# ruanjue/smartdenovo

Hardware: AMD Instinct MI355X
Metric: Gbp of candidate pairs aligned/sec (wtzmo all-vs-all) (higher is better)
Workload: dtype int32/int16

## Files before the change

smartdenovo_amd/csrc/wtz_tasks.h:

```cpp
#ifndef WTZ_TASKS_H
#define WTZ_TASKS_H

#include "wtz_sw.h"
#include "wtz_sw_wave.h"
#include "wtz_sw_grp.h"
#include "wtz_sw_lane.h"
#include "wtz_dotmatrix.h"

typedef struct {
	wtz_reads_t R; wtz_zindex_t Z; const wtz_params_t *P; wtz_pool_t *pool;
	wtz_zindex_t ZQ;
	uint32_t dm_first_big;
} wtz_env_t;

#define WTZ_WAVE_LDS_BYTES 8192
#ifndef WTZ_GAP_LDS_BYTES
#define WTZ_GAP_LDS_BYTES 12288
#endif
#ifndef WTZ_PAIR_LDS_BYTES
#define WTZ_PAIR_LDS_BYTES 8192
#endif
#ifndef WTZ_PAIR_DM_LDS_BYTES
#define WTZ_PAIR_DM_LDS_BYTES 24576
#endif
#if defined(__HIP_DEVICE_COMPILE__)
WTZ_D int32_t *wtz_wave_scratch(){ extern __shared__ int32_t wtz_dyn_lds[]; return wtz_dyn_lds; }
#else
WTZ_COOP_HOST int32_t *wtz_wave_scratch(){ return NULL; }
#endif

#if defined(WTZ_DEBUG_CRUMBS) && defined(__HIPCC__)
__device__ unsigned int *wtz_crumbs = NULL;
#endif
#if defined(WTZ_DEBUG_CRUMBS) && defined(__HIP_DEVICE_COMPILE__)
#define WTZ_CRUMB(t, code) do { if(wtz_crumbs && WTZ_LANE == 0) __hip_atomic_store(&wtz_crumbs[t], (unsigned int)(code), __ATOMIC_RELAXED, __HIP_MEMORY_SCOPE_SYSTEM); } while(0)
#else
#define WTZ_CRUMB(t, code) do { } while(0)
#endif
#define WTZ_PAIR_NEEDS_ZBIG (-3)
template<int ENGINE = -1, bool ZBIG = true>
WTZ_HD void wtz_task_pair(uint32_t t, const wtz_env_t &V, const uint32_t *qid, const uint32_t *cid, wtz_pairres_t *res){
	const wtz_params_t *P = V.P;
	const bool dm = ENGINE < 0 ? (P->dot_matrix != 0) : (ENGINE == 1);
	const uint32_t q = qid[t], c = cid[t];
	wtz_pairres_t r; memset(&r, 0, sizeof r);
	wtz_zhit_t *hits = NULL; uint32_t n = 0;
#if defined(__HIP_DEVICE_COMPILE__)
#define WTZ_TICK() ((uint64_t)clock64())
#else
#define WTZ_TICK() ((uint64_t)0)
#endif
	const uint64_t tk0 = WTZ_TICK();
	WTZ_CRUMB(t, 1);
	const bool aux = P->aux_strand != 0;
#if defined(__HIP_DEVICE_COMPILE__)
	const bool ok0 = wtz_zmatch_coop(V.ZQ, V.Z, q, c, V.R.rdlen[c], P->max_kmer_var, V.pool, &hits, &n, aux, (uint32_t*)wtz_wave_scratch(), dm ? (uint32_t)WTZ_PAIR_DM_LDS_BYTES : (uint32_t)WTZ_PAIR_LDS_BYTES);
#else
	const bool ok0 = wtz_zmatch_coop(V.ZQ, V.Z, q, c, V.R.rdlen[c], P->max_kmer_var, V.pool, &hits, &n, aux);
#endif
	const bool ok = wtz_coop_bcast32(ok0 ? 1u : 0u) != 0;
	n = wtz_coop_bcast32(n);
	hits = (wtz_zhit_t*)(uintptr_t)wtz_coop_bcast64((uint64_t)(uintptr_t)hits);
	const uint64_t tk1 = WTZ_TICK();
	WTZ_CRUMB(t, 2 | (n << 8));
	wtz_zhit_t *sorted = NULL;
#if defined(__HIP_DEVICE_COMPILE__)
	__threadfence_block();
	if(ok && (aux ? n > 0 : n * P->zsize >= P->ztot)){
		int pbad = 0;
		if(dm) sorted = wtz_sort_hits_wave<1>(hits, n, V.pool, (uint64_t*)wtz_wave_scratch(), WTZ_PAIR_DM_LDS_BYTES / 8, &pbad);
		else              sorted = wtz_sort_hits_wave<0>(hits, n, V.pool, (uint64_t*)wtz_wave_scratch(), WTZ_PAIR_LDS_BYTES / 8, &pbad);
		if(wtz_coop_bcast32((uint32_t)pbad)) r.bad = 1;
		sorted = (wtz_zhit_t*)(uintptr_t)wtz_coop_bcast64((uint64_t)(uintptr_t)sorted);
	}
#endif
	const uint32_t lane = WTZ_LANE;
	WTZ_CRUMB(t, 3 | (n << 8));
	if(!ok || r.bad){ r.bad = 1; if(lane == 0) res[t] = r; WTZ_CRUMB(t, 0xFF); return; }
	r.n_hits = n;
	if(aux ? n == 0 : n * P->zsize < P->ztot){ r.gate = 0; if(lane == 0) res[t] = r; WTZ_CRUMB(t, 0xFF); return; }
	r.gate = 1;
	if(dm){
		wtz_vec<wtz_zhit_t> cache; cache.a = sorted ? sorted : hits; cache.n = n; cache.cap = n + 2; cache.pool = V.pool; cache.bad = 0;
		const uint64_t tk2 = WTZ_TICK();
		uint64_t tkd = 0;
#if defined(__HIP_DEVICE_COMPILE__)
		uint8_t *dlds = (uint8_t*)wtz_wave_scratch();
#else
		static thread_local uint64_t emul_dm_lds[WTZ_PAIR_DM_LDS_BYTES / 8];
		uint8_t *dlds = (uint8_t*)emul_dm_lds;
#endif
		wtz_dm_result_t d = wtz_dot_matrix_align(cache, V.pool, (int32_t)V.R.rdlen[q], (int32_t)V.R.rdlen[c], P, &r.bad, sorted != NULL, &tkd, dlds, WTZ_PAIR_DM_LDS_BYTES, true, V.dm_first_big != 0);
		if(lane != 0) return;
		if(d.dir == -2){ r.anchors[0] = cache.a; r.nanchors[0] = cache.n; }
		r.dm_score = d.score; r.dm_qb = d.qb; r.dm_qe = d.qe; r.dm_tb = d.tb; r.dm_te = d.te; r.dm_dir = d.dir;
		{ const uint64_t tk3 = WTZ_TICK(); r.tick[0] = (uint32_t)((tk1 - tk0) >> 10); r.tick[1] = (uint32_t)((tk2 - tk1) >> 10); r.tick[2] = (uint32_t)((tkd - tk2) >> 10); r.tick[3] = (uint32_t)((tk3 - tk0) >> 10); }
		res[t] = r; return;
	}
	if(sorted) hits = sorted;
	else { WTZ_CRUMB(t, 4 | (n << 8)); if(lane == 0) wtz_sort_exact(hits, (size_t)n, wtz_gt_off12()); WTZ_WAVE_SYNC(); }
	WTZ_CRUMB(t, 5 | (n << 8));
	const uint64_t tk2 = WTZ_TICK();
	wtz_winscratch_t sc;
	{
		uint64_t pa = 0;
		if(lane == 0) pa = (uint64_t)(uintptr_t)wtz_pool_alloc(V.pool, (size_t)(n + 2) * (4 * 7 + 8 + sizeof(wtz_zhit_t)) + 16);
		pa = wtz_coop_bcast64(pa);
		sc.ts = (uint32_t*)(uintptr_t)pa;
	}
	if(sc.ts == NULL){ r.bad = 1; if(lane == 0) res[t] = r; WTZ_CRUMB(t, 0xFF); return; }
	sc.as = (int32_t*)(sc.ts + (n + 2)); sc.wb = sc.ts + 2 * (n + 2); sc.we = sc.ts + 3 * (n + 2); sc.wo = sc.ts + 4 * (n + 2); sc.wf = sc.ts + 5 * (n + 2); sc.wd = sc.ts + 6 * (n + 2);
	sc.tk = (uint64_t*)(sc.ts + 7 * (n + 2) + ((7 * (n + 2)) & 1)); sc.ztmp = (wtz_zhit_t*)(sc.tk + (n + 2));
#if defined(__HIP_DEVICE_COMPILE__)
	sc.lds = (uint64_t*)wtz_wave_scratch();
#else
	static thread_local uint64_t emul_lds[WTZ_PAIR_LDS_BYTES / 8];
	sc.lds = emul_lds;
#endif
	sc.lds_u64 = WTZ_PAIR_LDS_BYTES / 8;
	sc.big = NULL; sc.big_u64 = 0; sc.need_big = 0;
#ifndef WTZ_MERGE_SCALAR
	wtz_merge_prepare(hits, n, sc, P->kwin);
#endif
	for(uint32_t dir = 0; dir < 2; dir++){
		wtz_vec<wtz_win_t> wins; wtz_vec<wtz_zhit_t> anchors;
		wins.a = NULL; wins.n = wins.cap = 0; wins.pool = V.pool; wins.bad = 0;
		anchors.a = NULL; anchors.n = anchors.cap = 0; anchors.pool = V.pool; anchors.bad = 0;
		if(lane == 0){ wins.init(V.pool, 16); anchors.init(V.pool, n + 16); }
		WTZ_CRUMB(t, (6 + dir) | (n << 8));
		const unsigned long long ptm = WTZ_PROF_T(); (void)ptm;
#ifdef WTZ_MERGE_SCALAR
		const uint32_t nw = wtz_merge_windows_coop<ZBIG>(hits, n, dir, wins, anchors, sc, P->zsize, P->kwin, P->kstep, P->zovl);
#else
		const uint32_t nw = wtz_merge_windows_wave<ZBIG>(hits, n, dir, wins, anchors, sc, P->zsize, P->kwin, P->kstep, P->zovl);
#endif
		WTZ_PROF_ADD(63, ptm);
		if(!ZBIG && sc.need_big){
			if(lane == 0){ wtz_pairres_t r2; memset(&r2, 0, sizeof r2); r2.n_hits = r.n_hits; r2.gate = 1; r2.dm_dir = WTZ_PAIR_NEEDS_ZBIG; res[t] = r2; }
			WTZ_CRUMB(t, 0xFF);
			return;
		}
		WTZ_CRUMB(t, (8 + dir) | (n << 8));
		if(wtz_coop_bcast32((uint32_t)(wins.bad | anchors.bad))){ r.bad = 1; continue; }
		if(nw == 0) continue;
		const unsigned long long ptc = WTZ_PROF_T(); (void)ptc;
		WTZ_WAVE_SYNC();
		const uint32_t wn = wtz_coop_bcast32(wins.n);
		wtz_win_t *wa = (wtz_win_t*)(uintptr_t)wtz_coop_bcast64((uint64_t)(uintptr_t)wins.a);
		int32_t *mem = NULL;
		if(wn > 64u || WTZ_NLANES == 1u){
			uint64_t pa = 0;
			if(lane == 0) pa = (uint64_t)(uintptr_t)wtz_pool_alloc(V.pool, (size_t)wn * 8 + 8);
			mem = (int32_t*)(uintptr_t)wtz_coop_bcast64(pa);
			if(mem == NULL){ r.bad = 1; continue; }
		}
		r.ovl[dir] = WTZ_OVL29(wtz_chain_windows_wave(wa, wn, P->W, mem));
		if(r.ovl[dir] < P->ztot) continue;
		const uint32_t k = wtz_keep_chain_members(wa, wn);
		r.nwin[dir] = k; r.win[dir] = wa; r.anchors[dir] = anchors.a; r.nanchors[dir] = anchors.n;
		WTZ_PROF_ADD(62, ptc);
	}
	if(lane != 0) return;
	{ const uint64_t tk3 = WTZ_TICK(); r.tick[0] = (uint32_t)((tk1 - tk0) >> 10); r.tick[1] = (uint32_t)((tk2 - tk1) >> 10); r.tick[2] = (uint32_t)((tk3 - tk2) >> 10); r.tick[3] = (uint32_t)((tk3 - tk0) >> 10); }
	res[t] = r;
	WTZ_CRUMB(t, 0xFF);
}

WTZ_HD void wtz_task_pair_dm_big(uint32_t t, const wtz_env_t &V, const uint32_t *list, const uint32_t *qid, const uint32_t *cid, wtz_pairres_t *res, uint32_t lds_bytes, bool last, bool big){
	const wtz_params_t *P = V.P;
	const uint32_t pi = list[t], q = qid[pi], c = cid[pi];
	wtz_pairres_t r = res[pi];
	wtz_vec<wtz_zhit_t> cache; cache.a = r.anchors[0]; cache.n = r.nanchors[0]; cache.cap = cache.n + 2; cache.pool = V.pool; cache.bad = 0;
	uint64_t tkd = 0;
#if defined(__HIP_DEVICE_COMPILE__)
	uint8_t *dlds = (uint8_t*)wtz_wave_scratch();
	wtz_dm_result_t d = wtz_dot_matrix_align(cache, V.pool, (int32_t)V.R.rdlen[q], (int32_t)V.R.rdlen[c], P, &r.bad, true, &tkd, dlds, lds_bytes, !last, big);
#else
	(void)lds_bytes; (void)last; (void)big;
	wtz_dm_result_t d = wtz_dot_matrix_align(cache, V.pool, (int32_t)V.R.rdlen[q], (int32_t)V.R.rdlen[c], P, &r.bad, true, &tkd, (uint8_t*)NULL, 0, false, false);
#endif
	if(WTZ_LANE != 0) return;
	r.dm_score = d.score; r.dm_qb = d.qb; r.dm_qe = d.qe; r.dm_tb = d.tb; r.dm_te = d.te; r.dm_dir = d.dir;
	res[pi] = r;
}

typedef struct {
	uint32_t item;
	uint32_t widx;
} wtz_wintask_t;

typedef struct { wtz_aln_t x; uint32_t *cigar; uint32_t cigar_len; uint32_t pass; unsigned long long cells; } wtz_reg_t;

typedef struct {
	uint32_t q, c, dir;
	const wtz_win_t *win; const wtz_zhit_t *anchors; uint32_t nwin;
	wtz_reg_t *regs;
} wtz_alnitem_t;

typedef struct {
	wtz_aln_t x; uint32_t n_regs; uint32_t cigar_len; uint32_t *cigar; int32_t bad;
	unsigned long long cells_shift, cells_fixed, cells_global;
	uint32_t text_len;
} wtz_alnres_dev_t;

WTZ_HD uint32_t wtz_cigar_text_len(const uint32_t *c, uint32_t n){
	uint32_t k = 0;
	for(uint32_t i = 0; i < n; i++){ uint32_t len = c[i] >> 4; if(len == 0) continue; uint32_t d = 1; while(len >= 10){ len /= 10; d++; } k += d + 1; }
	return k;
}
WTZ_HD void wtz_cigar_text_write(const uint32_t *c, uint32_t n, char *s){
	uint32_t k = 0;
// ... 959 lines not shown
```

smartdenovo_amd/csrc/wtz_window.h:

```cpp
#ifndef WTZ_WINDOW_H
#define WTZ_WINDOW_H

#include "wtz_seed.h"

#define WTZ_KWIN_MAX_OFFSET_DEV 50

WTZ_HD bool wtz_zmatch(const wtz_zindex_t &ZQ, const wtz_zindex_t &ZC, uint32_t q, uint32_t c, uint32_t clen, uint32_t max_var, wtz_vec<wtz_zhit_t> &out, bool same_strand = false){
	const uint64_t qo = ZQ.zoff[q], co = ZC.zoff[c];
	const uint32_t cn = (uint32_t)(ZC.zoff[c + 1] - co), qd = ZQ.dn[q];
	const uint32_t *dmer = ZQ.dmer + qo;
	for(uint32_t k = 0; k < cn; k++){
		if(!ZC.ok[co + k]) continue;
		uint32_t m = ZC.mer[co + k];
		uint32_t lo = 0, hi = qd;
		while(lo < hi){ uint32_t mid = (lo + hi) >> 1; if(dmer[mid] < m) lo = mid + 1; else hi = mid; }
		if(lo >= qd || dmer[lo] != m) continue;
		uint32_t cpos = ZC.pos[co + k], clen2 = ZC.len[co + k];
		uint32_t first = ZQ.dfirst[qo + lo], cnt = ZQ.dcnt[qo + lo];
		for(uint32_t e = 0; e < cnt; e++){
			uint32_t qi = ZQ.sidx[qo + first + e];
			uint32_t qpos = ZQ.pos[qo + qi], qlen = ZQ.len[qo + qi];
			uint32_t dv = qlen > clen2 ? qlen - clen2 : clen2 - qlen;
			if(dv > max_var) continue;
			uint32_t d1 = qpos & 1u, d2 = cpos & 1u;
// ... 124 lines not shown
			}
			total += tot;
		}
	}
	if(lane == 0){ wtz_zhit_t z0; z0.o1 = z0.o2 = z0.ll = z0.gid = 0; hits[total] = z0; hits[total + 1] = z0; }
	*out = hits; *n_out = total;
	return true;
}

struct wtz_gt_off12 { WTZ_HDM bool operator()(const wtz_zhit_t &a, const wtz_zhit_t &b) const {
	uint64_t ka = ((uint64_t)ZH_OFF1(a) << 32) | ZH_OFF2(a), kb = ((uint64_t)ZH_OFF1(b) << 32) | ZH_OFF2(b); return ka > kb; } };
struct wtz_gt_off1 { WTZ_HDM bool operator()(const wtz_zhit_t &a, const wtz_zhit_t &b) const { return ZH_OFF1(a) > ZH_OFF1(b); } };
struct wtz_gt_idx_off2 { const wtz_zhit_t *rs; WTZ_HDM bool operator()(uint32_t a, uint32_t b) const { return ZH_OFF2(rs[a]) > ZH_OFF2(rs[b]); } };

#if defined(__HIP_DEVICE_COMPILE__)
template<int SH> struct wtz_gt_keybits { WTZ_HDM bool operator()(uint64_t a, uint64_t b) const { return (a >> SH) > (b >> SH); } };
template<int BYDIAG, bool W_LDS>
WTZ_D wtz_zhit_t *wtz_sort_hits_body(const wtz_zhit_t *hits, uint32_t n, wtz_pool_t *pool, uint64_t *lds, uint32_t lds_u64, uint64_t *w_pool, uint32_t np, int *pool_bad){
	const uint32_t lane = WTZ_LANE;
	const int SH = BYDIAG ? 15 : 16;
	uint64_t *w = W_LDS ? lds : w_pool;
	for(uint32_t i = lane; i < np; i += 64){
		uint64_t v = ~0ull;
		if(i < n){
			if(BYDIAG) v = ((uint64_t)((int64_t)ZH_OFF1(hits[i]) - (int64_t)ZH_OFF2(hits[i]) + (1 << 24)) << 39) | ((uint64_t)ZH_OFF1(hits[i]) << 15) | i;
			else       v = ((uint64_t)ZH_OFF1(hits[i]) << 40) | ((uint64_t)ZH_OFF2(hits[i]) << 16) | i;
		}
		w[i] = v;
	}
	__threadfence_block();
	if(W_LDS) wtz_coop_sort_u64(w, np);
	else {
		uint32_t ln = 128; while(lds && ln * 2 <= lds_u64) ln <<= 1;
		wtz_coop_sort_u64_windowed(w, np, lds, lds ? ln : 0);
	}
	uint32_t tie = 0;
	for(uint32_t i = lane; i + 1 < n; i += 64) if((w[i] >> SH) == (w[i + 1] >> SH)){
		if(BYDIAG) tie = 1;
		else { const wtz_zhit_t &a = hits[(uint32_t)(w[i] & 0xFFFFu)], &b = hits[(uint32_t)(w[i + 1] & 0xFFFFu)]; if(ZH_LEN1(a) != ZH_LEN1(b) || ZH_STRAND(a) == ZH_STRAND(b) || (i + 2 < n && (w[i] >> SH) == (w[i + 2] >> SH))) tie = 1; }
	}
	uint32_t any; (void)wtz_coop_excl_scan(tie, &any);
	if(any){
		if(!W_LDS) return NULL;
		for(uint32_t i = lane; i < n; i += 64){
			uint64_t v;
			if(BYDIAG) v = ((uint64_t)((int64_t)ZH_OFF1(hits[i]) - (int64_t)ZH_OFF2(hits[i]) + (1 << 24)) << 39) | ((uint64_t)ZH_OFF1(hits[i]) << 15) | i;
			else       v = ((uint64_t)ZH_OFF1(hits[i]) << 40) | ((uint64_t)ZH_OFF2(hits[i]) << 16) | i;
			w[i] = v;
		}
		__threadfence_block();
		if(lane == 0){ if(BYDIAG) wtz_sort_exact(w, (size_t)n, wtz_gt_keybits<15>()); else wtz_sort_exact(w, (size_t)n, wtz_gt_keybits<16>()); }
		__threadfence_block();
	}
	uint64_t oa = 0;
	if(lane == 0) oa = (uint64_t)(uintptr_t)wtz_pool_alloc(pool, (size_t)(n + 2) * sizeof(wtz_zhit_t));
	oa = wtz_coop_bcast64(oa);
	wtz_zhit_t *out = (wtz_zhit_t*)(uintptr_t)oa;
	if(out == NULL){ *pool_bad = 1; return NULL; }
	for(uint32_t i = lane; i < n; i += 64) out[i] = hits[(uint32_t)(w[i] & ((1u << SH) - 1u))];
	if(lane == 0){ wtz_zhit_t z0; z0.o1 = z0.o2 = z0.ll = z0.gid = 0; out[n] = z0; out[n + 1] = z0; }
	__threadfence_block();
	return out;
}
template<int BYDIAG>
WTZ_D wtz_zhit_t *wtz_sort_hits_wave(const wtz_zhit_t *hits, uint32_t n, wtz_pool_t *pool, uint64_t *lds, uint32_t lds_u64, int *pool_bad){
	const uint32_t lane = WTZ_LANE;
	*pool_bad = 0;
	if(n < 2 || n > (BYDIAG ? 32767u : 65535u)) return NULL;
	const int SH = BYDIAG ? 15 : 16;
	uint32_t np = 64; while(np < n) np <<= 1;
	uint64_t *w;
	if(lds && np <= lds_u64) w = lds;
	else {
		uint64_t a = 0;
		if(lane == 0) a = (uint64_t)(uintptr_t)wtz_pool_alloc(pool, (size_t)np * 8);
		a = wtz_coop_bcast64(a);
		w = (uint64_t*)(uintptr_t)a;
		if(w == NULL){ *pool_bad = 1; return NULL; }
	}
	return (w == lds) ? wtz_sort_hits_body<BYDIAG, true>(hits, n, pool, lds, lds_u64, w, np, pool_bad) : wtz_sort_hits_body<BYDIAG, false>(hits, n, pool, lds, lds_u64, w, np, pool_bad);
}
#endif

typedef struct { uint32_t *ts; int32_t *as; uint32_t *wb, *we, *wo; uint64_t *tk; wtz_zhit_t *ztmp; uint64_t *lds; uint32_t lds_u64; mutable uint64_t *big; mutable uint32_t big_u64; mutable uint32_t need_big; uint32_t *wf, *wd; } wtz_winscratch_t;
struct wtz_gt_hi32 { WTZ_HDM bool operator()(uint64_t a, uint64_t b) const { return (uint32_t)(a >> 32) > (uint32_t)(b >> 32); } };

typedef struct { uint32_t base, o1, o2, ll; } wtz_hitcur_t;
WTZ_HD void wtz_hitcur_get(wtz_hitcur_t &c, const wtz_zhit_t *rs, uint32_t lim, uint32_t i, uint32_t &o1, uint32_t &o2, uint32_t &ll){
	if(i - c.base >= WTZ_NLANES){
		c.base = i;
		const uint32_t idx = i + WTZ_LANE;
		if(idx <= lim){ const wtz_zhit_t h = rs[idx]; c.o1 = h.o1; c.o2 = h.o2; c.ll = h.ll; } else { c.o1 = c.o2 = c.ll = 0; }
	}
	const uint32_t l = i - c.base;
	o1 = wtz_coop_lane32(c.o1, l); o2 = wtz_coop_lane32(c.o2, l); ll = wtz_coop_lane32(c.ll, l);
}

#ifndef WTZ_SCAN_REST_FN
#define WTZ_SCAN_REST_FN WTZ_HD
#endif
#ifndef WTZ_SCAN_FN
#define WTZ_SCAN_FN WTZ_HD
#endif
template<bool K_LDS>
WTZ_SCAN_REST_FN uint32_t wtz_scan_windows_rest(const wtz_zhit_t *rs, uint32_t dir, uint32_t beg, uint32_t end, int32_t bound,
		wtz_vec<wtz_win_t> &wins, wtz_vec<wtz_zhit_t> &anchors, const wtz_winscratch_t &sc, uint32_t zsize, uint32_t kwin, uint32_t zovl, int32_t *max_e0, uint32_t n, unsigned long long pw0, uint64_t *KB){
	const uint32_t lane = WTZ_LANE;
	uint64_t *K = K_LDS ? sc.lds : KB;
	auto sort_keys = [&](uint64_t *w, uint32_t npw){
		if(K_LDS || sc.lds == NULL){ wtz_coop_sort_u64(w, npw); return; }
		uint32_t ln = 128; while(ln * 2 <= sc.lds_u64) ln <<= 1;
		wtz_coop_sort_u64_windowed(w, npw, sc.lds_u64 >= 128u ? sc.lds : NULL, ln);
	};
	uint32_t ret = 0; int32_t me0 = -0x7FFFFFFF;
	(void)pw0; (void)zsize;
	WTZ_PROF_ADD(16, pw0); WTZ_PROF_CNT(21, 1); WTZ_PROF_CNT(22, n);
	const unsigned long long pw1 = WTZ_PROF_T(); (void)pw1;
	uint32_t np = 64; while(np < n) np <<= 1;
	bool had_tie = false, exact = false;
	const uint32_t wins_n0 = wins.n, anchors_n0 = anchors.n;
retry_scan:
	if(exact){
		uint32_t m = 0;
		for(uint32_t b0 = beg; b0 < end; b0 += WTZ_NLANES){
			const uint32_t idx = b0 + lane;
			bool keep = false; uint32_t o2 = 0;
			if(idx < end){ const uint32_t o1 = rs[idx].o1; o2 = rs[idx].o2; keep = (((o1 ^ o2) >> 31) == dir) && ((int32_t)(o1 & 0x7FFFFFFFu) >= bound); }
			uint32_t tot; const uint32_t pos = wtz_coop_rank(keep, &tot);
			if(keep) K[m + pos] = ((uint64_t)(o2 & 0x7FFFFFFFu) << 32) | idx;
			m += tot;
		}
		WTZ_WAVE_SYNC();
		{ const unsigned long long px = WTZ_PROF_T(); (void)px; if(lane == 0) wtz_sort_exact(K, (size_t)n, wtz_gt_hi32()); WTZ_PROF_ADD(25, px); WTZ_PROF_CNT(24, 1000); }
		WTZ_WAVE_SYNC();
	} else {
#if defined(__HIP_DEVICE_COMPILE__)
	bool in_regs = false;
	if(n <= 64u){
		WTZ_WAVE_SYNC();
		const uint64_t v = wtz_wave_sort64(lane < n ? K[lane] : ~0ull);
		const uint32_t nhi = (uint32_t)__shfl_down((int)(uint32_t)(v >> 32), 1, 64);
		const bool tie = lane + 1 < n && (uint32_t)(v >> 32) == nhi;
		uint32_t any; (void)wtz_coop_rank(tie, &any);
		had_tie = any != 0;
		if(lane < n) K[lane] = v;
		WTZ_WAVE_SYNC();
		in_regs = true;
	}
	if(!in_regs)
#endif
	{
	for(uint32_t i = n + lane; i < np; i += WTZ_NLANES) K[i] = ~0ull;
	WTZ_WAVE_SYNC();
	sort_keys(K, np);
	bool tie = false;
	for(uint32_t i = lane; i + 1 < n; i += WTZ_NLANES) if((K[i] >> 32) == (K[i + 1] >> 32)) tie = true;
	uint32_t any; (void)wtz_coop_rank(tie, &any);
	had_tie = any != 0;
	}
	if(had_tie) WTZ_PROF_CNT(26, 1000);
	}
	WTZ_PROF_ADD(17, pw1);
	const unsigned long long pw2 = WTZ_PROF_T(); (void)pw2;
	wtz_zhit_t *S = (wtz_zhit_t*)(K + np);
	for(uint32_t x = lane; x < n; x += WTZ_NLANES) S[x] = rs[(uint32_t)K[x]];
	WTZ_WAVE_SYNC();
	WTZ_PROF_ADD(18, pw2);
	const unsigned long long pw3 = WTZ_PROF_T(); (void)pw3;
	unsigned long long pw4 = 0; (void)pw4;
	uint32_t n2_all = 0;
	{
		uint32_t *EP = (uint32_t*)K;
		uint32_t accA = 0, accE = 0, jrun = 0, n2 = 0;
		uint32_t lwo = 0, lwb_o2 = 0, lwe_o2 = 0;
		for(uint32_t c0 = 0; c0 < n; c0 += WTZ_NLANES){
			const uint32_t i = c0 + lane; const bool in = i < n;
			uint32_t o2 = 0, l2 = 0, e2 = 0, add = 0, ev = 0;
			if(in){
				const wtz_zhit_t p = S[i]; o2 = ZH_OFF2(p); l2 = ZH_LEN2(p); e2 = o2 + l2;
				uint32_t lst = 0; if(i){ const wtz_zhit_t q = S[i - 1]; lst = ZH_OFF2(q) + ZH_LEN2(q); }
				add = (o2 > lst) ? l2 : e2 - lst;
				if(i + 1 < n){ const uint32_t s1 = ZH_OFF2(S[i + 1]); ev = l2 - (s1 < e2 ? e2 - s1 : 0u); }
			}
			uint32_t totA, totE;
			const uint32_t exA = wtz_coop_excl_scan(add, &totA), exE = wtz_coop_excl_scan(ev, &totE);
			if(in) EP[i] = accE + exE;
			WTZ_WAVE_SYNC();
			uint32_t jm = 0;
			if(in){ uint32_t lo = 0, hi = i; while(lo < hi){ const uint32_t mid = (lo + hi) >> 1; if(e2 > ZH_OFF2(S[mid]) + kwin) lo = mid + 1; else hi = mid; } jm = lo; }
			jm = wtz_coop_incl_max32(jm); jm = jm > jrun ? jm : jrun;
			uint32_t ol = 0, jo2 = 0;
			if(in){ ol = accA + exA + add - EP[jm]; jo2 = ZH_OFF2(S[jm]); }
			const uint32_t lastl = (n - c0 < WTZ_NLANES ? n - c0 : WTZ_NLANES) - 1;
			accA += totA; accE += totE; jrun = wtz_coop_lane32(jm, lastl);
			unsigned long long fl = wtz_coop_ballot(in && ol >= zovl);
			while(fl){
				const uint32_t l = (uint32_t)__builtin_ctzll(fl); fl &= fl - 1;
				const uint32_t ol_ = wtz_coop_lane32(ol, l), o2_ = wtz_coop_lane32(o2, l), jo2_ = wtz_coop_lane32(jo2, l), j_ = wtz_coop_lane32(jm, l);
				if(n2 && (o2_ <= lwe_o2 + kwin / 3 || jo2_ <= lwb_o2 + kwin / 3)){
					if(ol_ > lwo){ if(lane == 0){ sc.wb[n2-1] = j_; sc.we[n2-1] = c0 + l; } lwo = ol_; lwb_o2 = jo2_; lwe_o2 = o2_; }
				} else { if(lane == 0){ sc.wb[n2] = j_; sc.we[n2] = c0 + l; } lwo = ol_; lwb_o2 = jo2_; lwe_o2 = o2_; n2++; }
			}
			WTZ_WAVE_SYNC();
		}
#ifdef WTZ_EXP_CNT_EMPTY
		WTZ_PROF_ADD(19, pw3); pw4 = WTZ_PROF_T(); WTZ_PROF_CNT(23, n2 == 0 ? 1 : 0);
#else
		WTZ_PROF_ADD(19, pw3); pw4 = WTZ_PROF_T(); WTZ_PROF_CNT(23, n2);
#endif
		n2_all = n2;
		if(had_tie && !exact){
			uint32_t cut = 0;
			if(lane == 0) for(uint32_t wq = 0; wq < n2; wq++){ const uint32_t we = sc.we[wq]; if(we + 1 < n && ZH_OFF2(S[we + 1]) == ZH_OFF2(S[we])) cut = 1; }
			if(wtz_coop_bcast32(cut)) n2_all = 0xFFFFFFFFu;
		}
	}
	if(n2_all == 0xFFFFFFFFu){ WTZ_PROF_CNT(28, 1000); exact = true; goto retry_scan; }
	int32_t last_end1 = 0; uint32_t last_ovl = 0;
	for(uint32_t wi = 0; wi < n2_all; wi++){
		uint32_t size = 0, cnt = 0, wb = 0, we = 0;
		uint64_t *ak = K;
		if(lane == 0){ size = anchors.n; wb = sc.wb[wi]; we = sc.we[wi]; }
		size = wtz_coop_bcast32(size); wb = wtz_coop_bcast32(wb); we = wtz_coop_bcast32(we);
		const uint32_t m = we - wb + 1;
		int32_t offset;
		WTZ_WAVE_SYNC();
#if defined(__HIP_DEVICE_COMPILE__)
		if(m <= 64u){
			uint32_t key = 0xFFFFFFFFu;
			if(lane < m){ const wtz_zhit_t p = S[wb + lane]; key = (uint32_t)((int32_t)ZH_OFF1(p) - (int32_t)ZH_OFF2(p)) ^ 0x80000000u; }
			key = wtz_wave_sort32(key);
			offset = (int32_t)(wtz_coop_lane32(key, m / 2) ^ 0x80000000u);
		} else
#endif
		{
			uint32_t mp = 64; while(mp < m) mp <<= 1;
			for(uint32_t x = lane; x < mp; x += WTZ_NLANES){
				uint64_t v = ~0ull;
				if(x < m){ const wtz_zhit_t p = S[wb + x]; v = (uint64_t)((uint32_t)((int32_t)ZH_OFF1(p) - (int32_t)ZH_OFF2(p)) ^ 0x80000000u); }
				ak[x] = v;
			}
			WTZ_WAVE_SYNC();
			sort_keys(ak, mp);
			offset = (int32_t)((uint32_t)ak[m / 2] ^ 0x80000000u);
			WTZ_WAVE_SYNC();
		}
		auto fill_members = [&]() -> uint32_t {
			uint32_t c2 = 0;
			for(uint32_t c0 = 0; c0 < m; c0 += WTZ_NLANES){
				const uint32_t j = wb + c0 + lane;
				bool keep = false; uint32_t o1 = 0;
				if(c0 + lane < m){ const wtz_zhit_t p = S[j]; const int32_t off = (int32_t)ZH_OFF1(p) - (int32_t)ZH_OFF2(p); o1 = ZH_OFF1(p); keep = !(off < offset - WTZ_KWIN_MAX_OFFSET_DEV || off > offset + WTZ_KWIN_MAX_OFFSET_DEV); }
				uint32_t tot; const uint32_t pos = wtz_coop_rank(keep, &tot);
				if(keep) ak[c2 + pos] = ((uint64_t)o1 << 32) | j;
				c2 += tot;
			}
			WTZ_WAVE_SYNC();
			return c2;
		};
		cnt = fill_members();
		if(cnt == 0) continue;
		{
			uint32_t any = 0;
#if defined(__HIP_DEVICE_COMPILE__)
			if(cnt <= 64u){
				const uint64_t v = wtz_wave_sort64(lane < cnt ? ak[lane] : ~0ull);
				const uint32_t nhi = (uint32_t)__shfl_down((int)(uint32_t)(v >> 32), 1, 64);
				const bool tie = lane + 1 < cnt && (uint32_t)(v >> 32) == nhi;
				(void)wtz_coop_rank(tie, &any);
				if(!any && lane < cnt) ak[lane] = v;
				WTZ_WAVE_SYNC();
			} else
#endif
			{
				uint32_t np2 = 64; while(np2 < cnt) np2 <<= 1;
				for(uint32_t i = cnt + lane; i < np2; i += WTZ_NLANES) ak[i] = ~0ull;
				WTZ_WAVE_SYNC();
				sort_keys(ak, np2);
				bool tie = false;
				for(uint32_t i = lane; i + 1 < cnt; i += WTZ_NLANES) if((ak[i] >> 32) == (ak[i + 1] >> 32)) tie = true;
				(void)wtz_coop_rank(tie, &any);
				WTZ_PROF_CNT(29, 1000);
				if(any){ WTZ_WAVE_SYNC(); (void)fill_members(); }
			}
			if(any){
				if(had_tie && !exact){
					if(lane == 0){ wins.n = wins_n0; anchors.n = anchors_n0; }
					ret = 0; me0 = -0x7FFFFFFF; exact = true;
					WTZ_PROF_CNT(30, 1000);
					goto retry_scan;
				}
				const unsigned long long px = WTZ_PROF_T(); (void)px;
				if(lane == 0) wtz_sort_exact(ak, (size_t)cnt, wtz_gt_hi32());
				WTZ_PROF_ADD(27, px); WTZ_PROF_CNT(31, 1000);
				WTZ_WAVE_SYNC();
			}
		}
		uint32_t stop = 0; uint64_t abase = 0;
		if(lane == 0){ if(!anchors.reserve(size + cnt)) stop = 1; else abase = (uint64_t)(uintptr_t)anchors.a; }
		if(wtz_coop_bcast32(stop)) break;
		abase = wtz_coop_bcast64(abase);
		wtz_zhit_t *A = (wtz_zhit_t*)(uintptr_t)abase + size;
		uint32_t ol = 0, b0 = 0x7FFFFFFFu, e0 = 0, b1 = 0x7FFFFFFFu, e1 = 0;
		for(uint32_t c0 = 0; c0 < cnt; c0 += WTZ_NLANES){
			const uint32_t k = c0 + lane; uint32_t add = 0;
			if(k < cnt){
				const wtz_zhit_t p = S[(uint32_t)ak[k]];
				A[k] = p;
				uint32_t lst = 0; if(k){ const wtz_zhit_t q = S[(uint32_t)ak[k - 1]]; lst = ZH_OFF1(q) + ZH_LEN1(q); }
				const uint32_t o1 = ZH_OFF1(p), x1 = o1 + ZH_LEN1(p), o2 = ZH_OFF2(p), x2 = o2 + ZH_LEN2(p);
				add = (o1 > lst) ? ZH_LEN1(p) : x1 - lst;
				b0 = o1 < b0 ? o1 : b0; e0 = x1 > e0 ? x1 : e0; b1 = o2 < b1 ? o2 : b1; e1 = x2 > e1 ? x2 : e1;
			}
			uint32_t tot; (void)wtz_coop_excl_scan(add, &tot); ol += tot;
		}
		b0 = wtz_coop_min32(b0); b1 = wtz_coop_min32(b1); e0 = ~wtz_coop_min32(~e0); e1 = ~wtz_coop_min32(~e1);
		if(ol * 2 < zovl) continue;
		if(ret && ((int32_t)e1 <= (int32_t)((uint32_t)last_end1 + kwin / 3) && ol <= last_ovl)) continue;
		if(lane == 0){
			wtz_win_t w;
			w.pb2 = 0; w.closed = 0; w.dir = (uint8_t)dir; w.pad = 0;
			w.beg[0] = (int32_t)b0; w.beg[1] = (int32_t)b1; w.end[0] = (int32_t)e0; w.end[1] = (int32_t)e1;
			anchors.n = size + cnt;
			w.anchors[0] = size; w.anchors[1] = anchors.n;
			w.ovl = WTZ_OVL29(ol);
			if(!wins.push(w)) stop = 1;
		}
		if(wtz_coop_bcast32(stop)) break;
		ret++;
		last_end1 = (int32_t)e1; last_ovl = WTZ_OVL29(ol);
		if(me0 < (int32_t)e0) me0 = (int32_t)e0;
		WTZ_WAVE_SYNC();
	}
	WTZ_PROF_ADD(20, pw4);
	WTZ_WAVE_SYNC();
	*max_e0 = (int32_t)wtz_coop_bcast32((uint32_t)me0);
	return wtz_coop_bcast32(ret);
}

WTZ_DN uint32_t wtz_scan_windows_rest_pool(const wtz_zhit_t *rs, uint32_t dir, uint32_t beg, uint32_t end, int32_t bound,
		wtz_vec<wtz_win_t> &wins, wtz_vec<wtz_zhit_t> &anchors, const wtz_winscratch_t &sc, uint32_t zsize, uint32_t kwin, uint32_t zovl, int32_t *max_e0, uint32_t n, unsigned long long pw0, uint64_t *KB){
	return wtz_scan_windows_rest<false>(rs, dir, beg, end, bound, wins, anchors, sc, zsize, kwin, zovl, max_e0, n, pw0, KB);
}

template<bool ZBIG>
WTZ_SCAN_FN uint32_t wtz_scan_windows_coop(const wtz_zhit_t *rs, uint32_t dir, uint32_t beg, uint32_t end, int32_t bound,
		wtz_vec<wtz_win_t> &wins, wtz_vec<wtz_zhit_t> &anchors, const wtz_winscratch_t &sc, uint32_t zsize, uint32_t kwin, uint32_t zovl, int32_t *max_e0){
	const uint32_t lane = WTZ_LANE;
	uint64_t *K = sc.lds;
	uint32_t n = 0;
	beg = wtz_coop_bcast32(beg); end = wtz_coop_bcast32(end); bound = (int32_t)wtz_coop_bcast32((uint32_t)bound); dir = wtz_coop_bcast32(dir);
	zsize = wtz_coop_bcast32(zsize); kwin = wtz_coop_bcast32(kwin); zovl = wtz_coop_bcast32(zovl);
	const unsigned long long pw0 = WTZ_PROF_T(); (void)pw0;
	constexpr uint32_t RC = 4;
#ifndef WTZ_NO_SCAN_CACHE
	const bool cached = (K != NULL) && (end - beg <= WTZ_NLANES * RC) && (sc.lds_u64 >= (WTZ_NLANES * RC > 64u ? WTZ_NLANES * RC : 64u) + 2u * WTZ_NLANES * RC + 2u);
#else
	const bool cached = false;
#endif
	if(cached){
		uint32_t q2[RC]; uint32_t kpm = 0;
		#pragma unroll
		for(uint32_t c = 0; c < RC; c++){
			const uint32_t idx = beg + c * WTZ_NLANES + lane;
			q2[c] = 0;
			if(idx < end){ const uint32_t o1 = rs[idx].o1, o2 = rs[idx].o2; q2[c] = o2 & 0x7FFFFFFFu; if((((o1 ^ o2) >> 31) == dir) && ((int32_t)(o1 & 0x7FFFFFFFu) >= bound)) kpm |= 1u << c; }
		}
		n = 0;
		#pragma unroll
		for(uint32_t c = 0; c < RC; c++) n += (uint32_t)__builtin_popcountll(wtz_coop_ballot((kpm >> c) & 1u));
		if(n * zsize < zovl){ WTZ_PROF_ADD(12, pw0); WTZ_PROF_CNT(7, 1); return 0; }
#ifndef WTZ_NO_SCAN_PRECHECK
		{
			uint32_t mn = 0xFFFFFFFFu, mx = 0;
			#pragma unroll
			for(uint32_t c = 0; c < RC; c++) if((kpm >> c) & 1u){ mn = q2[c] < mn ? q2[c] : mn; mx = q2[c] > mx ? q2[c] : mx; }
			mn = wtz_coop_min32(mn); mx = ~wtz_coop_min32(~mx);
			const uint32_t bw = kwin >= 8 ? kwin / 8 : 1;
			const uint32_t nadj = (kwin - 1) / bw + 2;
			const uint32_t nb = (mx - mn) / bw + 1 + nadj;
			if(nb <= sc.lds_u64 * 2){
				uint32_t *B = (uint32_t*)K;
				for(uint32_t b = lane; b < nb; b += WTZ_NLANES) B[b] = 0;
				WTZ_WAVE_SYNC();
				#pragma unroll
				for(uint32_t c = 0; c < RC; c++) if((kpm >> c) & 1u){
					const uint32_t bin = (q2[c] - mn) / bw, l2 = rs[beg + c * WTZ_NLANES + lane].ll >> 16;
#if defined(__HIP_DEVICE_COMPILE__)
					atomicAdd(&B[bin], l2);
#else
					B[bin] += l2;
#endif
				}
				WTZ_WAVE_SYNC();
				uint32_t best = 0;
				for(uint32_t b = lane; b + nadj <= nb; b += WTZ_NLANES){ uint32_t v = 0; for(uint32_t t = 0; t < nadj; t++) v += B[b + t]; best = v > best ? v : best; }
				best = ~wtz_coop_min32(~best);
				WTZ_WAVE_SYNC();
				if(best < zovl){ WTZ_PROF_CNT(23, 0); WTZ_PROF_ADD(12, pw0); WTZ_PROF_CNT(7, 1); return 0; }
			}
		}
#endif
		uint32_t m = 0;
		#pragma unroll
		for(uint32_t c = 0; c < RC; c++){
			const bool kp = (kpm >> c) & 1u;
			uint32_t tot; const uint32_t pos = wtz_coop_rank(kp, &tot);
			if(kp) K[m + pos] = ((uint64_t)q2[c] << 32) | (beg + c * WTZ_NLANES + lane);
			m += tot;
		}
	}
	for(int pass = 0; pass < 2 && !cached; pass++){
		n = 0;
		for(uint32_t b0 = beg; b0 < end; b0 += WTZ_NLANES){
			const uint32_t idx = b0 + lane;
			bool keep = false; uint32_t o2 = 0;
			if(idx < end){ const uint32_t o1 = rs[idx].o1; o2 = rs[idx].o2; keep = (((o1 ^ o2) >> 31) == dir) && ((int32_t)(o1 & 0x7FFFFFFFu) >= bound); }
			uint32_t tot; const uint32_t pos = wtz_coop_rank(keep, &tot);
			if(pass && keep) K[n + pos] = ((uint64_t)(o2 & 0x7FFFFFFFu) << 32) | idx;
			n += tot;
		}
		if(pass) break;
		if(n * zsize < zovl){ WTZ_PROF_ADD(12, pw0); WTZ_PROF_CNT(7, 1); return 0; }
#ifndef WTZ_NO_SCAN_PRECHECK
		if(K != NULL){
			uint32_t mn = 0xFFFFFFFFu, mx = 0;
			for(uint32_t b0 = beg; b0 < end; b0 += WTZ_NLANES){
				const uint32_t idx = b0 + lane;
				if(idx < end){ const uint32_t o1 = rs[idx].o1, o2 = rs[idx].o2; if((((o1 ^ o2) >> 31) == dir) && ((int32_t)(o1 & 0x7FFFFFFFu) >= bound)){ const uint32_t f = o2 & 0x7FFFFFFFu; mn = f < mn ? f : mn; mx = f > mx ? f : mx; } }
			}
			mn = wtz_coop_min32(mn); mx = ~wtz_coop_min32(~mx);
			const uint32_t bw = kwin >= 8 ? kwin / 8 : 1;
			const uint32_t nadj = (kwin - 1) / bw + 2;
			const uint32_t nb = (mx - mn) / bw + 1 + nadj;
			if(nb <= sc.lds_u64 * 2){
				uint32_t *B = (uint32_t*)K;
				for(uint32_t b = lane; b < nb; b += WTZ_NLANES) B[b] = 0;
				WTZ_WAVE_SYNC();
				for(uint32_t b0 = beg; b0 < end; b0 += WTZ_NLANES){
					const uint32_t idx = b0 + lane;
					if(idx < end){
						const uint32_t o1 = rs[idx].o1, o2 = rs[idx].o2;
						if((((o1 ^ o2) >> 31) == dir) && ((int32_t)(o1 & 0x7FFFFFFFu) >= bound)){
							const uint32_t bin = ((o2 & 0x7FFFFFFFu) - mn) / bw, l2 = rs[idx].ll >> 16;
#if defined(__HIP_DEVICE_COMPILE__)
							atomicAdd(&B[bin], l2);
#else
							B[bin] += l2;
#endif
						}
					}
				}
				WTZ_WAVE_SYNC();
				uint32_t best = 0;
				for(uint32_t b = lane; b + nadj <= nb; b += WTZ_NLANES){ uint32_t v = 0; for(uint32_t t = 0; t < nadj; t++) v += B[b + t]; best = v > best ? v : best; }
				best = ~wtz_coop_min32(~best);
				WTZ_WAVE_SYNC();
				if(best < zovl){ WTZ_PROF_CNT(23, 0); WTZ_PROF_ADD(12, pw0); WTZ_PROF_CNT(7, 1); return 0; }
			}
		}
#endif
		uint32_t np0 = 64; while(np0 < n) np0 <<= 1;
		if(K == NULL || np0 + 2 * n + 2 > sc.lds_u64){
			if(!ZBIG){ sc.need_big = 1; *max_e0 = -0x7FFFFFFF; return 0; }
			const uint32_t need = np0 + 2 * n + 2;
#ifndef WTZ_PAIR_NO_POOL_SCAN
			if(sc.big_u64 < need){
				const uint32_t cap = need > 2 * sc.big_u64 ? need : 2 * sc.big_u64;
				uint64_t pa = 0;
				if(lane == 0) pa = (uint64_t)(uintptr_t)wtz_pool_alloc(wins.pool, (size_t)cap * 8 + 16);
				pa = wtz_coop_bcast64(pa);
				if(pa){ sc.big = (uint64_t*)(uintptr_t)pa; sc.big_u64 = cap; }
			}
#endif
#ifdef WTZ_PAIR_NO_POOL_SCAN
			if(false){
#else
			if(sc.big_u64 >= need){
#endif
				uint64_t *KB = sc.big; uint32_t m = 0;
				for(uint32_t b0 = beg; b0 < end; b0 += WTZ_NLANES){
					const uint32_t idx = b0 + lane;
					bool keep = false; uint32_t o2 = 0;
					if(idx < end){ const uint32_t o1 = rs[idx].o1; o2 = rs[idx].o2; keep = (((o1 ^ o2) >> 31) == dir) && ((int32_t)(o1 & 0x7FFFFFFFu) >= bound); }
					uint32_t tot; const uint32_t pos = wtz_coop_rank(keep, &tot);
					if(keep) KB[m + pos] = ((uint64_t)(o2 & 0x7FFFFFFFu) << 32) | idx;
					m += tot;
				}
				if constexpr(ZBIG){
					const uint32_t r = wtz_scan_windows_rest_pool(rs, dir, beg, end, bound, wins, anchors, sc, zsize, kwin, zovl, max_e0, n, pw0, KB);
					*max_e0 = (int32_t)wtz_coop_bcast32((uint32_t)*max_e0);
					return wtz_coop_bcast32(r);
				}
			} else {
				if(lane == 0) wins.bad = 1;
				*max_e0 = -0x7FFFFFFF;
				return 0;
			}
		}
	}
	return wtz_scan_windows_rest<true>(rs, dir, beg, end, bound, wins, anchors, sc, zsize, kwin, zovl, max_e0, n, pw0, NULL);
}

template<bool ZBIG>
WTZ_HD uint32_t wtz_merge_windows_coop(const wtz_zhit_t *rs, uint32_t n_rs, uint32_t dir, wtz_vec<wtz_win_t> &wins, wtz_vec<wtz_zhit_t> &anchors,
		const wtz_winscratch_t &sc, uint32_t zsize, uint32_t kwin, uint32_t kstep, uint32_t zovl){
	n_rs = wtz_coop_bcast32(n_rs); dir = wtz_coop_bcast32(dir); zsize = wtz_coop_bcast32(zsize); kwin = wtz_coop_bcast32(kwin); kstep = wtz_coop_bcast32(kstep); zovl = wtz_coop_bcast32(zovl);
	const uint32_t P_off1 = 0x1FFFFFu, P_len1 = 0x3FFu, lim = n_rs + 1;
	uint32_t i, j, n, ol, ol2, lst, wlst, s, t, ret, o1, o2, ll;
	uint32_t p_off1, p_len1, p0_off1, p0_len1, p1_off1, p1_len1;
	int32_t nxt;
	wtz_hitcur_t ci, cj; ci.base = cj.base = 0x80000000u; ci.o1 = ci.o2 = ci.ll = cj.o1 = cj.o2 = cj.ll = 0;
	ol = 0; lst = 0; wlst = 0; ret = 0;
	for(j = 0; j < n_rs; j++){ wtz_hitcur_get(cj, rs, lim, j, o1, o2, ll); if(((o1 ^ o2) >> 31) ^ dir) continue; break; }
	if(j == n_rs) return 0;
	wtz_hitcur_get(cj, rs, lim, j, o1, o2, ll);
	p0_off1 = o1 & 0x7FFFFFFFu; p0_len1 = ll & 0xFFFFu;
	p_off1 = p_len1 = 0;
	for(i = j; i <= n_rs; i++){
		if(i < n_rs){
			wtz_hitcur_get(ci, rs, lim, i, o1, o2, ll);
			if(((o1 ^ o2) >> 31) ^ dir) continue;
			p_off1 = o1 & 0x7FFFFFFFu; p_len1 = ll & 0xFFFFu;
		} else { p_off1 = P_off1; p_len1 = P_len1; }
		if(p_off1 > p0_off1 + kwin){
			if(ol >= zovl){
				int32_t me0 = 0;
				n = wtz_scan_windows_coop<ZBIG>(rs, dir, j, i, (int32_t)wlst, wins, anchors, sc, zsize, kwin, zovl, &me0);
				if(!ZBIG && sc.need_big) return 0;
				if(n){
					if((int32_t)wlst < me0 + 20) wlst = (uint32_t)(me0 + 20);
					ret += n;
					p0_off1 = p_off1; p0_len1 = p_len1; ol = p_len1; lst = p_off1 + p_len1; j = i;
				} else {
					nxt = (int32_t)(p0_off1 + kstep);
					while((int32_t)p0_off1 < nxt && j < i){
						++j; wtz_hitcur_get(cj, rs, lim, j, o1, o2, ll); p1_off1 = o1 & 0x7FFFFFFFu; p1_len1 = ll & 0xFFFFu;
						s = WTZ_MAX(p0_off1, p1_off1);
						t = WTZ_MIN(p0_off1 + p0_len1, p1_off1 + p1_len1);
						ol2 = s < t ? t - s : 0;
						ol = ol + ol2 - p0_len1;
						p0_off1 = p1_off1; p0_len1 = p1_len1;
					}
				}
			}
			if(p_off1 == P_off1) break;
			while(p_off1 > p0_off1 + kwin){
				++j; wtz_hitcur_get(cj, rs, lim, j, o1, o2, ll); p1_off1 = o1 & 0x7FFFFFFFu; p1_len1 = ll & 0xFFFFu;
				s = WTZ_MAX(p0_off1, p1_off1);
				t = WTZ_MIN(p0_off1 + p0_len1, p1_off1 + p1_len1);
				ol2 = s < t ? t - s : 0;
				ol = ol + ol2 - p0_len1;
				p0_off1 = p1_off1; p0_len1 = p1_len1;
			}
		} else {
			if(p_off1 >= lst) ol += p_len1;
			else if((int32_t)(p_off1 + p_len1) > (int32_t)lst) ol += p_off1 + p_len1 - lst;
			else continue;
			lst = p_off1 + p_len1;
		}
	}
	return ret;
}

#if defined(__HIP_DEVICE_COMPILE__)
WTZ_D uint32_t wtz_coop_excl_max32(uint32_t v){ const uint32_t in = wtz_coop_incl_max32(v); const uint32_t up = (uint32_t)__shfl_up((int)in, 1, 64); return WTZ_LANE ? up : 0u; }
WTZ_D uint32_t wtz_coop_all_max32(uint32_t v){ return (uint32_t)__builtin_amdgcn_readlane((int)wtz_coop_incl_max32(v), 63); }
WTZ_D uint32_t wtz_coop_first_lane(unsigned long long m){ return (uint32_t)__builtin_amdgcn_readfirstlane((int)__builtin_ctzll(m)); }
#else
WTZ_COOP_HOST uint32_t wtz_coop_excl_max32(uint32_t){ return 0u; }
WTZ_COOP_HOST uint32_t wtz_coop_all_max32(uint32_t v){ return v; }
WTZ_COOP_HOST uint32_t wtz_coop_first_lane(unsigned long long){ return 0u; }
#endif

WTZ_HD void wtz_merge_prepare(const wtz_zhit_t *rs, uint32_t n_rs, const wtz_winscratch_t &sc, uint32_t kwin){
	const uint32_t lane = WTZ_LANE;
	n_rs = wtz_coop_bcast32(n_rs); kwin = wtz_coop_bcast32(kwin);
	uint32_t f_carry = 0, d_carry = 0;
	for(uint32_t b0 = 0; b0 < n_rs; b0 += WTZ_NLANES){
		const uint32_t i = b0 + lane; const bool in = i < n_rs;
		uint32_t a = 0, l = 0, a1 = 0, l1 = 0;
		if(in){ a = ZH_OFF1(rs[i]); l = ZH_LEN1(rs[i]); a1 = ZH_OFF1(rs[i + 1]); l1 = ZH_LEN1(rs[i + 1]); }
		uint32_t lo = f_carry, hi = in ? i : f_carry;
		while(wtz_coop_ballot(lo < hi) != 0ull){
// ... 192 lines not shown
```

Baseline: 10.68.

## Stage hit fields and window bounds in LDS; shrink per-pair scratch allocation

In the cached scan path, the hit fields o1/o2/ll are copied into a region at the top of the wave's LDS scratch on the first global read. The later gather into S and the histogram pass then read LDS instead of re-reading global hits. Window begin/end pairs go into spare LDS slots below that region when they fit and fall back to global arrays otherwise. The per-pair pool scratch shrinks from seven arrays plus tk/ztmp to four arrays, and the anchors vector is reserved lazily on first use instead of eagerly per direction. The cost is more complex LDS capacity bookkeeping with fallback branches, and a risk of overlap bugs if the capacity checks are wrong.

```diff
diff --git a/smartdenovo_amd/csrc/wtz_tasks.h b/smartdenovo_amd/csrc/wtz_tasks.h
--- a/smartdenovo_amd/csrc/wtz_tasks.h
+++ b/smartdenovo_amd/csrc/wtz_tasks.h
@@ -104,13 +104,12 @@
 	wtz_winscratch_t sc;
 	{
 		uint64_t pa = 0;
-		if(lane == 0) pa = (uint64_t)(uintptr_t)wtz_pool_alloc(V.pool, (size_t)(n + 2) * (4 * 7 + 8 + sizeof(wtz_zhit_t)) + 16);
+		if(lane == 0) pa = (uint64_t)(uintptr_t)wtz_pool_alloc(V.pool, (size_t)(n + 2) * (4 * 4) + 16);
 		pa = wtz_coop_bcast64(pa);
-		sc.ts = (uint32_t*)(uintptr_t)pa;
-	}
-	if(sc.ts == NULL){ r.bad = 1; if(lane == 0) res[t] = r; WTZ_CRUMB(t, 0xFF); return; }
-	sc.as = (int32_t*)(sc.ts + (n + 2)); sc.wb = sc.ts + 2 * (n + 2); sc.we = sc.ts + 3 * (n + 2); sc.wo = sc.ts + 4 * (n + 2); sc.wf = sc.ts + 5 * (n + 2); sc.wd = sc.ts + 6 * (n + 2);
-	sc.tk = (uint64_t*)(sc.ts + 7 * (n + 2) + ((7 * (n + 2)) & 1)); sc.ztmp = (wtz_zhit_t*)(sc.tk + (n + 2));
+		sc.wf = (uint32_t*)(uintptr_t)pa;
+	}
+	if(sc.wf == NULL){ r.bad = 1; if(lane == 0) res[t] = r; WTZ_CRUMB(t, 0xFF); return; }
+	sc.wd = sc.wf + (n + 2); sc.wb = sc.wf + 2 * (n + 2); sc.we = sc.wf + 3 * (n + 2); sc.nall = n;
 #if defined(__HIP_DEVICE_COMPILE__)
 	sc.lds = (uint64_t*)wtz_wave_scratch();
 #else
@@ -126,7 +125,6 @@
 		wtz_vec<wtz_win_t> wins; wtz_vec<wtz_zhit_t> anchors;
 		wins.a = NULL; wins.n = wins.cap = 0; wins.pool = V.pool; wins.bad = 0;
 		anchors.a = NULL; anchors.n = anchors.cap = 0; anchors.pool = V.pool; anchors.bad = 0;
-		if(lane == 0){ wins.init(V.pool, 16); anchors.init(V.pool, n + 16); }
 		WTZ_CRUMB(t, (6 + dir) | (n << 8));
 		const unsigned long long ptm = WTZ_PROF_T(); (void)ptm;
 #ifdef WTZ_MERGE_SCALAR
diff --git a/smartdenovo_amd/csrc/wtz_window.h b/smartdenovo_amd/csrc/wtz_window.h
--- a/smartdenovo_amd/csrc/wtz_window.h
+++ b/smartdenovo_amd/csrc/wtz_window.h
@@ -230,7 +230,7 @@
 }
 #endif
 
-typedef struct { uint32_t *ts; int32_t *as; uint32_t *wb, *we, *wo; uint64_t *tk; wtz_zhit_t *ztmp; uint64_t *lds; uint32_t lds_u64; mutable uint64_t *big; mutable uint32_t big_u64; mutable uint32_t need_big; uint32_t *wf, *wd; } wtz_winscratch_t;
+typedef struct { uint32_t *wb, *we; uint32_t nall; uint64_t *lds; uint32_t lds_u64; mutable uint64_t *big; mutable uint32_t big_u64; mutable uint32_t need_big; uint32_t *wf, *wd; } wtz_winscratch_t;
 struct wtz_gt_hi32 { WTZ_HDM bool operator()(uint64_t a, uint64_t b) const { return (uint32_t)(a >> 32) > (uint32_t)(b >> 32); } };
 
 typedef struct { uint32_t base, o1, o2, ll; } wtz_hitcur_t;
@@ -252,7 +252,8 @@
 #endif
 template<bool K_LDS>
 WTZ_SCAN_REST_FN uint32_t wtz_scan_windows_rest(const wtz_zhit_t *rs, uint32_t dir, uint32_t beg, uint32_t end, int32_t bound,
-		wtz_vec<wtz_win_t> &wins, wtz_vec<wtz_zhit_t> &anchors, const wtz_winscratch_t &sc, uint32_t zsize, uint32_t kwin, uint32_t zovl, int32_t *max_e0, uint32_t n, unsigned long long pw0, uint64_t *KB){
+		wtz_vec<wtz_win_t> &wins, wtz_vec<wtz_zhit_t> &anchors, const wtz_winscratch_t &sc, uint32_t zsize, uint32_t kwin, uint32_t zovl, int32_t *max_e0, uint32_t n, unsigned long long pw0, uint64_t *KB,
+		const uint32_t *R = NULL, uint32_t ktop = 0){
 	const uint32_t lane = WTZ_LANE;
 	uint64_t *K = K_LDS ? sc.lds : KB;
 	auto sort_keys = [&](uint64_t *w, uint32_t npw){
@@ -265,6 +266,9 @@
 	WTZ_PROF_ADD(16, pw0); WTZ_PROF_CNT(21, 1); WTZ_PROF_CNT(22, n);
 	const unsigned long long pw1 = WTZ_PROF_T(); (void)pw1;
 	uint32_t np = 64; while(np < n) np <<= 1;
+	const uint32_t wcap = (K_LDS && ktop > np + 2 * n + 2) ? ktop - (np + 2 * n + 2) : 0u;
+	auto put_win = [&](uint32_t w, uint32_t b, uint32_t e){ if(w < wcap) K[ktop - 1u - w] = ((uint64_t)e << 32) | b; else { sc.wb[w] = b; sc.we[w] = e; } };
+	auto get_win = [&](uint32_t w, uint32_t &b, uint32_t &e){ if(w < wcap){ const uint64_t v = K[ktop - 1u - w]; b = (uint32_t)v; e = (uint32_t)(v >> 32); } else { b = sc.wb[w]; e = sc.we[w]; } };
 	bool had_tie = false, exact = false;
 	const uint32_t wins_n0 = wins.n, anchors_n0 = anchors.n;
 retry_scan:
@@ -311,6 +315,10 @@
 	WTZ_PROF_ADD(17, pw1);
 	const unsigned long long pw2 = WTZ_PROF_T(); (void)pw2;
 	wtz_zhit_t *S = (wtz_zhit_t*)(K + np);
+	if(K_LDS && R != NULL){
+		const uint32_t rng = end - beg;
+		for(uint32_t x = lane; x < n; x += WTZ_NLANES){ const uint32_t k = (uint32_t)K[x] - beg; wtz_zhit_t h; h.o1 = R[k]; h.o2 = R[rng + k]; h.ll = R[2u * rng + k]; h.gid = 0; S[x] = h; }
+	} else
 	for(uint32_t x = lane; x < n; x += WTZ_NLANES) S[x] = rs[(uint32_t)K[x]];
 	WTZ_WAVE_SYNC();
 	WTZ_PROF_ADD(18, pw2);
@@ -346,8 +354,8 @@
 				const uint32_t l = (uint32_t)__builtin_ctzll(fl); fl &= fl - 1;
 				const uint32_t ol_ = wtz_coop_lane32(ol, l), o2_ = wtz_coop_lane32(o2, l), jo2_ = wtz_coop_lane32(jo2, l), j_ = wtz_coop_lane32(jm, l);
 				if(n2 && (o2_ <= lwe_o2 + kwin / 3 || jo2_ <= lwb_o2 + kwin / 3)){
-					if(ol_ > lwo){ if(lane == 0){ sc.wb[n2-1] = j_; sc.we[n2-1] = c0 + l; } lwo = ol_; lwb_o2 = jo2_; lwe_o2 = o2_; }
-				} else { if(lane == 0){ sc.wb[n2] = j_; sc.we[n2] = c0 + l; } lwo = ol_; lwb_o2 = jo2_; lwe_o2 = o2_; n2++; }
+					if(ol_ > lwo){ if(lane == 0) put_win(n2 - 1, j_, c0 + l); lwo = ol_; lwb_o2 = jo2_; lwe_o2 = o2_; }
+				} else { if(lane == 0) put_win(n2, j_, c0 + l); lwo = ol_; lwb_o2 = jo2_; lwe_o2 = o2_; n2++; }
 			}
 			WTZ_WAVE_SYNC();
 		}
@@ -359,7 +367,7 @@
 		n2_all = n2;
 		if(had_tie && !exact){
 			uint32_t cut = 0;
-			if(lane == 0) for(uint32_t wq = 0; wq < n2; wq++){ const uint32_t we = sc.we[wq]; if(we + 1 < n && ZH_OFF2(S[we + 1]) == ZH_OFF2(S[we])) cut = 1; }
+			if(lane == 0) for(uint32_t wq = 0; wq < n2; wq++){ uint32_t wb, we; get_win(wq, wb, we); if(we + 1 < n && ZH_OFF2(S[we + 1]) == ZH_OFF2(S[we])) cut = 1; }
 			if(wtz_coop_bcast32(cut)) n2_all = 0xFFFFFFFFu;
 		}
 	}
@@ -368,7 +376,7 @@
 	for(uint32_t wi = 0; wi < n2_all; wi++){
 		uint32_t size = 0, cnt = 0, wb = 0, we = 0;
 		uint64_t *ak = K;
-		if(lane == 0){ size = anchors.n; wb = sc.wb[wi]; we = sc.we[wi]; }
+		if(lane == 0){ size = anchors.n; get_win(wi, wb, we); }
 		size = wtz_coop_bcast32(size); wb = wtz_coop_bcast32(wb); we = wtz_coop_bcast32(we);
 		const uint32_t m = we - wb + 1;
 		int32_t offset;
@@ -445,7 +453,7 @@
 			}
 		}
 		uint32_t stop = 0; uint64_t abase = 0;
-		if(lane == 0){ if(!anchors.reserve(size + cnt)) stop = 1; else abase = (uint64_t)(uintptr_t)anchors.a; }
+		if(lane == 0){ if(anchors.cap == 0) (void)anchors.reserve(sc.nall + 16); if(!anchors.reserve(size + cnt)) stop = 1; else abase = (uint64_t)(uintptr_t)anchors.a; }
 		if(wtz_coop_bcast32(stop)) break;
 		abase = wtz_coop_bcast64(abase);
 		wtz_zhit_t *A = (wtz_zhit_t*)(uintptr_t)abase + size;
@@ -506,13 +514,20 @@
 #else
 	const bool cached = false;
 #endif
+	const uint32_t rng = end - beg;
+	uint32_t *R = NULL; uint32_t ktop = sc.lds_u64;
 	if(cached){
 		uint32_t q2[RC]; uint32_t kpm = 0;
+		R = (uint32_t*)K + 2u * sc.lds_u64 - 3u * rng; ktop = sc.lds_u64 - (3u * rng + 1u) / 2u;
 		#pragma unroll
 		for(uint32_t c = 0; c < RC; c++){
-			const uint32_t idx = beg + c * WTZ_NLANES + lane;
+			const uint32_t k = c * WTZ_NLANES + lane, idx = beg + k;
 			q2[c] = 0;
-			if(idx < end){ const uint32_t o1 = rs[idx].o1, o2 = rs[idx].o2; q2[c] = o2 & 0x7FFFFFFFu; if((((o1 ^ o2) >> 31) == dir) && ((int32_t)(o1 & 0x7FFFFFFFu) >= bound)) kpm |= 1u << c; }
+			if(idx < end){
+				const uint32_t o1 = rs[idx].o1, o2 = rs[idx].o2, ll = rs[idx].ll;
+				R[k] = o1; R[rng + k] = o2; R[2u * rng + k] = ll;
+				q2[c] = o2 & 0x7FFFFFFFu; if((((o1 ^ o2) >> 31) == dir) && ((int32_t)(o1 & 0x7FFFFFFFu) >= bound)) kpm |= 1u << c;
+			}
 		}
 		n = 0;
 		#pragma unroll
@@ -529,11 +544,12 @@
 			const uint32_t nb = (mx - mn) / bw + 1 + nadj;
 			if(nb <= sc.lds_u64 * 2){
 				uint32_t *B = (uint32_t*)K;
+				if(nb > ktop * 2){ R = NULL; ktop = sc.lds_u64; }
 				for(uint32_t b = lane; b < nb; b += WTZ_NLANES) B[b] = 0;
 				WTZ_WAVE_SYNC();
 				#pragma unroll
 				for(uint32_t c = 0; c < RC; c++) if((kpm >> c) & 1u){
-					const uint32_t bin = (q2[c] - mn) / bw, l2 = rs[beg + c * WTZ_NLANES + lane].ll >> 16;
+					const uint32_t bin = (q2[c] - mn) / bw, l2 = (R ? R[2u * rng + c * WTZ_NLANES + lane] : rs[beg + c * WTZ_NLANES + lane].ll) >> 16;
 #if defined(__HIP_DEVICE_COMPILE__)
 					atomicAdd(&B[bin], l2);
 #else
@@ -557,6 +573,7 @@
 			if(kp) K[m + pos] = ((uint64_t)q2[c] << 32) | (beg + c * WTZ_NLANES + lane);
 			m += tot;
 		}
+		if(R){ uint32_t np0 = 64; while(np0 < n) np0 <<= 1; if(np0 + 2 * n + 2 > ktop){ R = NULL; ktop = sc.lds_u64; } }
 	}
 	for(int pass = 0; pass < 2 && !cached; pass++){
 		n = 0;
@@ -647,7 +664,7 @@
 			}
 		}
 	}
-	return wtz_scan_windows_rest<true>(rs, dir, beg, end, bound, wins, anchors, sc, zsize, kwin, zovl, max_e0, n, pw0, NULL);
+	return wtz_scan_windows_rest<true>(rs, dir, beg, end, bound, wins, anchors, sc, zsize, kwin, zovl, max_e0, n, pw0, NULL, R, ktop);
 }
 
 template<bool ZBIG>
```

After: 10.74, median of 2. No clear change (+0.5%).
